# FeggieBoss/raytracing-course

Measured on AMD Instinct MI355X. Metric: Mray/s (closest-hit queries/s), dragon stand-in 1080p/256 spp, RAY_DEPTH 6, higher is better.
Workload: dtype f32

## Files before the change

raytracing-course_amd/csrc/device/pt_core.h:

```cpp
#pragma once
#include <stdint.h>

#if defined(__HIPCC__)
#include <hip/hip_runtime.h>
#define PT_HD __host__ __device__ __forceinline__
#else
#include <math.h>
#define PT_HD inline
#endif

namespace pt {

#if defined(__HIP_DEVICE_COMPILE__)
__device__ __forceinline__ bool pt_any(bool p) { return __ballot(p) != 0ull; }
#else
inline bool pt_any(bool p) { return p; }
#endif

struct f3 { float x, y, z; };
struct alignas(16) F4 { float x, y, z, w; };

PT_HD f3 mk3(float x, float y, float z) { f3 r; r.x = x; r.y = y; r.z = z; return r; }
PT_HD f3 operator+(f3 a, f3 b) { return mk3(a.x + b.x, a.y + b.y, a.z + b.z); }
PT_HD f3 operator-(f3 a, f3 b) { return mk3(a.x - b.x, a.y - b.y, a.z - b.z); }
PT_HD f3 operator*(f3 a, f3 b) { return mk3(a.x * b.x, a.y * b.y, a.z * b.z); }
PT_HD f3 operator/(f3 a, f3 b) { return mk3(a.x / b.x, a.y / b.y, a.z / b.z); }
PT_HD f3 operator*(float k, f3 a) { return mk3(k * a.x, k * a.y, k * a.z); }
PT_HD f3 operator*(f3 a, float k) { return mk3(a.x * k, a.y * k, a.z * k); }
PT_HD f3 operator/(f3 a, float k) { return mk3(a.x / k, a.y / k, a.z / k); }
PT_HD float dot(f3 a, f3 b) { return a.x * b.x + a.y * b.y + a.z * b.z; }
PT_HD f3 cross(f3 a, f3 b) { return mk3(a.y * b.z - b.y * a.z, a.z * b.x - b.z * a.x, a.x * b.y - b.x * a.y); }
PT_HD float fsqrt(float x) { return sqrtf(x); }
PT_HD f3 normalize(f3 v) { return v * (1.f / fsqrt(dot(v, v))); }
PT_HD float length(f3 v) { return fsqrt(dot(v, v)); }
PT_HD float smin(float a, float b) { return (b < a) ? b : a; }
PT_HD float smax(float a, float b) { return (a < b) ? b : a; }
PT_HD float fabs_(float a) { return fabsf(a); }

struct q4 { float x, y, z, w; };
PT_HD q4 conj(q4 q) { q4 r; r.x = -q.x; r.y = -q.y; r.z = -q.z; r.w = q.w; return r; }
PT_HD f3 qrot(q4 q, f3 v) {
    const f3 qv = mk3(q.x, q.y, q.z);
    const f3 uv = cross(qv, v);
    const f3 uuv = cross(qv, uv);
    return v + ((uv * q.w) + uuv) * 2.f;
}

#define PT_INF 1e18f
#define PT_PI_F 3.14159274101257324f

PT_HD uint32_t f2u(float f) { union { float f; uint32_t u; } c; c.f = f; return c.u; }
PT_HD float u2f(uint32_t u) { union { float f; uint32_t u; } c; c.u = u; return c.f; }

struct LogfEntry { double invc, logc; };
#if defined(__HIP_DEVICE_COMPILE__)
#define PT_TABLE __constant__
#else
#define PT_TABLE
#endif
PT_TABLE static const LogfEntry kLogfT[16] = {
    {0x1.661ec79f8f3bep+0, -0x1.57bf7808caadep-2}, {0x1.571ed4aaf883dp+0, -0x1.2bef0a7c06ddbp-2},
    {0x1.49539f0f010bp+0, -0x1.01eae7f513a67p-2},  {0x1.3c995b0b80385p+0, -0x1.b31d8a68224e9p-3},
    {0x1.30d190c8864a5p+0, -0x1.6574f0ac07758p-3}, {0x1.25e227b0b8eap+0, -0x1.1aa2bc79c81p-3},
    {0x1.1bb4a4a1a343fp+0, -0x1.a4e76ce8c0e5ep-4}, {0x1.12358f08ae5bap+0, -0x1.1973c5a611cccp-4},
    {0x1.0953f419900a7p+0, -0x1.252f438e10c1ep-5}, {0x1p+0, 0x0p+0},
    {0x1.e608cfd9a47acp-1, 0x1.aa5aa5df25984p-5},  {0x1.ca4b31f026aap-1, 0x1.c5e53aa362eb4p-4},
    {0x1.b2036576afce6p-1, 0x1.526e57720db08p-3},  {0x1.9c2d163a1aa2dp-1, 0x1.bc2860d22477p-3},
    {0x1.886e6037841edp-1, 0x1.1058bc8a07ee1p-2},  {0x1.767dcf5534862p-1, 0x1.4043057b6ee09p-2}};
PT_HD float logf_glibc(float x) {
    const double Ln2 = 0x1.62e42fefa39efp-1;
    const double A0 = -0x1.00ea348b88334p-2, A1 = 0x1.5575b0be00b6ap-2, A2 = -0x1.ffffef20a4123p-2;
    uint32_t ix = f2u(x);
    if (ix == 0x3f800000u) return 0.f;
    if (ix - 0x00800000u >= 0x7f800000u - 0x00800000u) {
        ix = f2u(x * 0x1p23f);
        ix -= 23u << 23;
    }
    const uint32_t tmp = ix - 0x3f330000u;
    const int i = (int)((tmp >> (23 - 4)) % 16u);
    const int k = (int32_t)tmp >> 23;
    const uint32_t iz = ix - (tmp & (0x1ffu << 23));
    const double invc = kLogfT[i].invc, logc = kLogfT[i].logc;
    const double z = (double)u2f(iz);
    const double r = z * invc - 1.0;
    const double y0 = logc + (double)k * Ln2;
    const double r2 = r * r;
    double y = A1 * r + A2;
    y = A0 * r2 + y;
    y = y * r2 + (y0 + r);
    return (float)y;
}

PT_HD double pow5_cr(double x) {
    const double x2 = x * x;
    const double h4 = x2 * x2;
    const double l4 = fma(x2, x2, -h4);
    const double h5 = h4 * x;
    const double e5 = fma(h4, x, -h5);
    return h5 + (e5 + l4 * x);
}

struct Rng {
    uint32_t x;
    float saved;
    uint32_t saved_ok;
};
PT_HD Rng rng_seed(uint32_t seed) {
    Rng r;
    const uint32_t s = seed % 2147483647u;
    r.x = (s == 0u) ? 1u : s;
    r.saved = 0.f;
    r.saved_ok = 0u;
    return r;
}
PT_HD uint32_t rng_next(Rng& r) {
    const uint64_t p = (uint64_t)r.x * 48271u;
    uint32_t v = (uint32_t)(p & 0x7fffffffu) + (uint32_t)(p >> 31);
    v = (v & 0x7fffffffu) + (v >> 31);
    if (v == 0x7fffffffu) v = 0u;
    r.x = v;
    return v;
}
PT_HD float rng_uniform(Rng& r) {
    const float sum = (float)(rng_next(r) - 1u);
    float u = sum / 2147483648.0f;
    if (u >= 1.0f) u = 0x1.fffffep-1f;
    return u * 1.0f + 0.0f;
}
PT_HD float rng_normal(Rng& r) {
    if (r.saved_ok) { r.saved_ok = 0u; return r.saved * 1.0f + 0.0f; }
    float a, b, r2;
    do {
        a = (float)((double)(2.0f * rng_uniform(r)) - 1.0);
        b = (float)((double)(2.0f * rng_uniform(r)) - 1.0);
        r2 = a * a + b * b;
    } while (r2 > 1.0f || r2 == 0.0f);
    const float m = fsqrt(-2.0f * logf_glibc(r2) / r2);
    r.saved = a * m;
    r.saved_ok = 1u;
    return b * m * 1.0f + 0.0f;
}

enum : uint32_t { T_PLANE = 1, T_BOX = 2, T_ELLIPSOID = 4, T_TRIANGLE = 8 };
enum : uint32_t { M_DIFFUSE = 0, M_METALLIC = 1, M_DIELECTRIC = 2 };

struct Node { F4 a, b; };
struct AuxNode { F4 a, b, c, d; };
#define PT_NODE_INTERIOR 0x80000000u
struct Prim { F4 p0, p1, p2, p3, p4; };
struct Shade { F4 s0, s1; };

struct SceneView {
    const Node* nodes;
    const AuxNode* aux;
    const Prim* prims;
    const Shade* shade;
    const uint32_t* planes;
    const uint32_t* emitters;
    uint32_t n_planes, n_emitters;
    f3 bg;
    float box_extent;
    const uint32_t* anc_info;
    const uint32_t* anc;
    const F4* blob;
    uint32_t o_nodes, o_aux, o_ainfo, o_anc, o_qprim, o_prim, o_bundle;
    uint32_t aux_rshift;
    float inv_emitters;
};

struct Ray { f3 o, d; };
struct Hit { float t; f3 n; uint32_t interior; };

PT_HD bool isect_plane(const Ray& r, f3 n, Hit& h) {
    const float dn = dot(r.d, n);
    const float t = -dot(r.o, n) / dn;
    if (t > 1e5f) return false;
    if (t > 0.f) {
        if (dn >= 0.f) { h.t = t; h.n = -1.f * n; h.interior = 1u; return true; }
        h.t = t; h.n = n; h.interior = 0u;
        return true;
    }
    return false;
}

PT_HD bool slab(f3 o, f3 d, f3 s, float& t, uint32_t& interior) {
    const f3 t1xyz = (-1.f * s - o) / d;
    const f3 t2xyz = (s - o) / d;
    const float t1x = smin(t1xyz.x, t2xyz.x), t2x = smax(t1xyz.x, t2xyz.x);
    const float t1y = smin(t1xyz.y, t2xyz.y), t2y = smax(t1xyz.y, t2xyz.y);
    const float t1z = smin(t1xyz.z, t2xyz.z), t2z = smax(t1xyz.z, t2xyz.z);
    const float t1 = smax(smax(t1x, t1y), t1z);
    const float t2 = smin(smin(t2x, t2y), t2z);
    if (t1 > t2) return false;
    if (t2 < 0.f) return false;
    interior = (t1 < 0.f) ? 1u : 0u;
    t = interior ? t2 : t1;
    return true;
}

PT_HD bool isect_box(const Ray& r, f3 s, Hit& h) {
    float t;
    uint32_t in;
    if (!slab(r.o, r.d, s, t, in)) return false;
    const f3 p = r.o + t * r.d;
    f3 n = p / s;
    if (in) n = -1.f * n;
    const float ax = fabs_(n.x), ay = fabs_(n.y), az = fabs_(n.z);
    float mx = ax;
    if (mx < ay) mx = ay;
    if (mx < az) mx = az;
    if (ax != mx) n.x = 0.f;
    if (ay != mx) n.y = 0.f;
    if (az != mx) n.z = 0.f;
    h.t = t; h.n = normalize(n); h.interior = in;
    return true;
}

PT_HD bool ellipsoid_root(const Ray& r, f3 rad, float& t, uint32_t& in) {
    const float a = dot(r.d / rad, r.d / rad);
    const float b = 2.f * dot(r.o / rad, r.d / rad);
    const float c = dot(r.o / rad, r.o / rad) - 1.f;
    const float d = b * b - 4.f * a * c;
    if (d <= 0.f) return false;
    const double sd = sqrt((double)d);
    float x1 = (float)(((double)-b - sd) / (double)(2.f * a));
    float x2 = (float)(((double)-b + sd) / (double)(2.f * a));
    if (x1 > x2) { const float tt = x1; x1 = x2; x2 = tt; }
    if (x2 < 0.f) return false;
    in = (x1 < 0.f) ? 1u : 0u;
    t = in ? x2 : x1;
    return true;
}
PT_HD bool isect_ellipsoid(const Ray& r, f3 rad, Hit& h) {
    float t;
    uint32_t in;
    if (!ellipsoid_root(r, rad, t, in)) return false;
    const f3 p = r.o + t * r.d;
    f3 n = normalize(p / (rad * rad));
    if (in) n = -1.f * n;
    h.t = t; h.n = n; h.interior = in;
    return true;
}

PT_HD bool isect_triangle_n(const Ray& r, f3 a, f3 b, f3 c, f3 n, Hit& h) {
    Hit ph;
    if (!isect_plane(r, n, ph)) return false;
    const f3 p = r.o + ph.t * r.d;
    if (!(dot(cross(b - a, p - a), n) > 0.f)) return false;
    if (!(dot(cross(p - a, c - a), n) > 0.f)) return false;
    if (!(dot(cross(c - b, p - b), n) > 0.f)) return false;
    h = ph;
    return true;
}
PT_HD bool isect_triangle(const Ray& r, f3 a, f3 b, f3 c, Hit& h) {
    return isect_triangle_n(r, a, b, c, normalize(cross(b - a, c - a)), h);
}

PT_HD bool prim_intersect(const Prim& P, const Ray& ray, Hit& h) {
    const f3 pos = mk3(P.p0.x, P.p0.y, P.p0.z);
    const uint32_t type = f2u(P.p0.w);
    q4 q; q.x = P.p1.x; q.y = P.p1.y; q.z = P.p1.z; q.w = P.p1.w;
    const q4 cq = conj(q);
    Ray lr;
    lr.o = qrot(cq, ray.o + -1.f * pos);
    lr.d = qrot(cq, ray.d);
    const f3 a = mk3(P.p2.x, P.p2.y, P.p2.z);
    bool ok;
    if (type == T_TRIANGLE) {
        ok = isect_triangle(lr, a, mk3(P.p3.x, P.p3.y, P.p3.z), mk3(P.p3.w, P.p4.x, P.p4.y), h);
    } else if (type == T_PLANE) {
        ok = isect_plane(lr, a, h);
    } else if (type == T_BOX) {
        ok = isect_box(lr, a, h);
    } else {
        ok = isect_ellipsoid(lr, a, h);
    }
    if (ok) h.n = normalize(qrot(q, h.n));
    return ok;
}

PT_HD bool bvh_prim_intersect(const Prim& P, const Ray& ray, Hit& h) {
    const f3 pos = mk3(P.p0.x, P.p0.y, P.p0.z);
    const uint32_t type = f2u(P.p0.w);
    q4 q; q.x = P.p1.x; q.y = P.p1.y; q.z = P.p1.z; q.w = P.p1.w;
    const q4 cq = conj(q);
    Ray lr;
    lr.o = qrot(cq, ray.o + -1.f * pos);
    lr.d = qrot(cq, ray.d);
    const f3 a = mk3(P.p2.x, P.p2.y, P.p2.z);
    bool ok;
    if (type == T_TRIANGLE) {
        ok = isect_triangle(lr, a, mk3(P.p3.x, P.p3.y, P.p3.z), mk3(P.p3.w, P.p4.x, P.p4.y), h);
    } else if (type == T_BOX) {
        ok = isect_box(lr, a, h);
    } else {
        ok = isect_ellipsoid(lr, a, h);
    }
    if (ok) h.n = normalize(qrot(q, h.n));
    return ok;
}

PT_HD bool plane_intersect(const Prim& P, const Ray& ray, Hit& h) {
    const f3 pos = mk3(P.p0.x, P.p0.y, P.p0.z);
    q4 q; q.x = P.p1.x; q.y = P.p1.y; q.z = P.p1.z; q.w = P.p1.w;
    const q4 cq = conj(q);
    Ray lr;
    lr.o = qrot(cq, ray.o + -1.f * pos);
    lr.d = qrot(cq, ray.d);
    if (!isect_plane(lr, mk3(P.p2.x, P.p2.y, P.p2.z), h)) return false;
    h.n = normalize(qrot(q, h.n));
    return true;
}

PT_HD f3 normal01_vec(Rng& R) {
    const float f1 = rng_normal(R);
    const float f2 = rng_normal(R);
    const float f3_ = rng_normal(R);
    return normalize(mk3(f1, f2, f3_));
}
PT_HD f3 sample_cosine(Rng& R, f3 n) {
    f3 dir = normal01_vec(R);
    dir = dir + n;
    if (dot(dir, n) <= 1e-8f) return n;
    if ((double)length(dir) <= 1e-4) return n;
    return normalize(dir);
}
PT_HD float pdf_cosine(f3 n, f3 d) { return smax(0.f, 1.f / PT_PI_F * dot(d, n)); }

PT_HD int points_for_pdf(const Prim& P, f3 x, f3 d, Hit& h1, Hit& h2) {
    Ray r; r.o = x; r.d = d;
    if (!prim_intersect(P, r, h1)) return 0;
    const float t = h1.t;
    if ((double)t <= 1e-8) return 0;
    const float eps = 1e-4f;
    Ray r2; r2.o = x + (t + eps) * d; r2.d = d;
    if (!prim_intersect(P, r2, h2)) return 1;
    h2.t += t + eps;
    return 2;
}

PT_HD f3 sample_box(Rng& R, const Prim& B, f3 x) {
    const f3 s = mk3(B.p2.x, B.p2.y, B.p2.z);
    const float wx = s.x * s.x, wy = s.y * s.y, wz = s.z * s.z;
    const f3 pos = mk3(B.p0.x, B.p0.y, B.p0.z);
    q4 q; q.x = B.p1.x; q.y = B.p1.y; q.z = B.p1.z; q.w = B.p1.w;
    for (;;) {
        float u = rng_uniform(R);
        const float side = (rng_uniform(R) <= 0.5f) ? 1.f : -1.f;
        u *= wx + wy + wz;
        float c1 = rng_uniform(R);
        float c2 = rng_uniform(R);
        float c3 = rng_uniform(R);
        c1 = 2.f * c1 - 1.f;
        c2 = 2.f * c2 - 1.f;
        c3 = 2.f * c3 - 1.f;
        f3 pnt = mk3(c1 * s.x, c2 * s.y, c3 * s.z);
        if (u < wx) pnt.x = side * s.x;
        else if (u < wx + wy) pnt.y = side * s.y;
        else pnt.z = side * s.z;
        const f3 on_box = qrot(q, pnt) + pos;
        const f3 smp = normalize(on_box - x);
        Hit h;
        Ray r; r.o = x; r.d = smp;
        if (prim_intersect(B, r, h)) return smp;
    }
}
PT_HD float pdf_point_box(const Prim& B, float dist2, f3 n, f3 d) {
    const float wx = B.p2.x * B.p2.x, wy = B.p2.y * B.p2.y, wz = B.p2.z * B.p2.z;
    const float p_y = 1.f / (8.f * (wx + wy + wz));
    return (p_y * dist2) / fabs_(dot(d, n));
}
PT_HD float pdf_box(const Prim& B, f3 x, f3 d) {
    Hit h1, h2;
    const int k = points_for_pdf(B, x, d, h1, h2);
    if (k == 0) return 1e-9f;
    const f3 cp = x + h1.t * d;
    float sum = pdf_point_box(B, dot(x - cp, x - cp), h1.n, d);
    if (k == 2) {
        const f3 op = x + h2.t * d;
        sum += pdf_point_box(B, dot(x - op, x - op), h2.n, d);
    }
    return sum;
}
PT_HD f3 sample_ellipsoid(Rng& R, const Prim& E, f3 x) {
    const f3 rr = mk3(E.p2.x, E.p2.y, E.p2.z);
    const f3 pos = mk3(E.p0.x, E.p0.y, E.p0.z);
    q4 q; q.x = E.p1.x; q.y = E.p1.y; q.z = E.p1.z; q.w = E.p1.w;
    for (;;) {
        const f3 k = normal01_vec(R);
        const f3 on = qrot(q, rr * k) + pos;
        const f3 smp = normalize(on - x);
        Hit h;
        Ray r; r.o = x; r.d = smp;
        if (prim_intersect(E, r, h)) return smp;
    }
}
PT_HD float pdf_point_ellipsoid(const Prim& E, float dist2, f3 y, f3 n_, f3 d) {
    const f3 rr = mk3(E.p2.x, E.p2.y, E.p2.z);
    const f3 pos = mk3(E.p0.x, E.p0.y, E.p0.z);
    q4 q; q.x = E.p1.x; q.y = E.p1.y; q.z = E.p1.z; q.w = E.p1.w;
    const f3 n = qrot(conj(q), y - pos) / rr;
    const float p_y = 1.f / (4.f * PT_PI_F * length(mk3(n.x * rr.y * rr.z, rr.x * n.y * rr.z, rr.x * rr.y * n.z)));
    return (p_y * dist2) / fabs_(dot(d, n_));
}
PT_HD float pdf_ellipsoid(const Prim& E, f3 x, f3 d) {
    Hit h1, h2;
    const int k = points_for_pdf(E, x, d, h1, h2);
    if (k == 0) return 1e-9f;
    const f3 cp = x + h1.t * d;
    float sum = pdf_point_ellipsoid(E, dot(x - cp, x - cp), cp, h1.n, d);
    if (k == 2) {
        const f3 op = x + h2.t * d;
        sum += pdf_point_ellipsoid(E, dot(x - op, x - op), op, h2.n, d);
    }
    return sum;
}
struct EmitGlobal {
    const SceneView& S;
    PT_HD Prim operator()(uint32_t k) const { return S.prims[S.emitters[k]]; }
};
template <class EM>
PT_HD f3 sample_mix_e(const SceneView& S, const EM& em, Rng& R, f3 x, f3 n) {
    const float flip = rng_uniform(R);
    if (S.n_emitters == 0u || flip <= 0.5f) return sample_cosine(R, n);
    const float fid = rng_uniform(R);
    const uint32_t id = (uint32_t)floorf(fid * (float)S.n_emitters);
    const Prim E = em(id);
    return f2u(E.p0.w) == T_BOX ? sample_box(R, E, x) : sample_ellipsoid(R, E, x);
}
PT_HD f3 sample_mix(const SceneView& S, Rng& R, f3 x, f3 n) { return sample_mix_e(S, EmitGlobal{S}, R, x, n); }
template <class EM>
PT_HD float pdf_mix_e(const SceneView& S, const EM& em, f3 x, f3 n, f3 d) {
    float sum = pdf_cosine(n, d);
    if (S.n_emitters != 0u) {
        float ps = 0.f;
        for (uint32_t k = 0; k < S.n_emitters; ++k) {
            const Prim E = em(k);
            ps += f2u(E.p0.w) == T_BOX ? pdf_box(E, x, d) : pdf_ellipsoid(E, x, d);
        }
        ps *= S.inv_emitters;
        sum = 0.5f * sum + 0.5f * ps;
    }
    return sum;
}
PT_HD float pdf_mix(const SceneView& S, f3 x, f3 n, f3 d) { return pdf_mix_e(S, EmitGlobal{S}, x, n, d); }

PT_HD f3 reflect(f3 n, f3 dir) { return dir - (2.0f * n) * dot(n, dir); }

PT_HD float saturate1(float v) { return smax(smin(1.f, v), 0.f); }
PT_HD float aces1(float x) {
    const float a = 2.51f, b = 0.03f, c = 2.43f, d = 0.59f, e = 0.14f;
    return saturate1((x * (a * x + b)) / (x * (c * x + d) + e));
}
PT_HD uint32_t quantize_gamma(float v, const float* thr) {
    uint32_t lo = 0;
    for (uint32_t step = 128; step >= 1; step >>= 1)
        if (thr[lo + step - 1] <= v) lo += step;
    return lo;
}

}
```

raytracing-course_amd/csrc/device/pt_trace.h:

```cpp
#pragma once
#include "pt_core.h"

namespace pt {

struct Counts {
    uint64_t rays;
    uint64_t nodes;
    uint64_t ptests;
    uint64_t planes;
    uint64_t aux;
    uint64_t fallbacks;
    uint32_t errs;
};

struct CamView {
    f3 pos, right, up, fwd;
    float tx, ty;
    float W, H;
};

PT_HD Ray camera_ray(const CamView& c, float x, float y) {
    const float nx = (2.f * x / c.W - 1.f) * c.tx;
    const float ny = -1.f * (2.f * y / c.H - 1.f) * c.ty;
    Ray r;
    r.o = c.pos;
    r.d = nx * c.right + ny * c.up + 1.f * c.fwd;
    return r;
}

#define PT_HITLIST 6

template <class Stack>
PT_HD int bvh_exact(const SceneView& S, const Ray& ray, float cb, Stack& stk, Hit& best, Counts& C) {
    int best_id = -1;
    best.t = PT_INF;
    float ms_t[PT_HITLIST];
    uint32_t ms_q[PT_HITLIST];
    uint32_t msn = 0;
    uint32_t nh = 0;
    uint32_t sp = 0;
    uint32_t node = 0;
    for (;;) {
        const Node nd = S.nodes[node];
        C.nodes++;
        const f3 c = mk3(nd.a.x, nd.a.y, nd.a.z);
        const f3 s = mk3(nd.a.w, nd.b.x, nd.b.y);
        float t;
        uint32_t interior;
        const bool hit = slab(ray.o + -1.f * c, ray.d, s, t, interior);
        bool descend = false;
        if (hit && !(cb < t && !interior)) {
            const uint32_t ref = f2u(nd.b.z), cnt = f2u(nd.b.w);
            if (!(cnt & PT_NODE_INTERIOR)) {
                Hit lb;
                lb.t = PT_INF;
                int lid = -1;
                for (uint32_t i = ref; i < ref + cnt; ++i) {
                    Hit h;
                    C.ptests++;
                    if (prim_intersect(S.prims[i], ray, h) && h.t < lb.t) { lb = h; lid = (int)i; }
                }
                if (lid >= 0) {
                    uint32_t keep = 0;
#pragma unroll
                    for (int k = 0; k < PT_HITLIST; ++k)
                        if ((uint32_t)k < msn && ms_t[k] < lb.t) keep = (uint32_t)k + 1u;
                    if (keep == PT_HITLIST) {
#pragma unroll
                        for (int k = 0; k + 1 < PT_HITLIST; ++k) { ms_t[k] = ms_t[k + 1]; ms_q[k] = ms_q[k + 1]; }
                        keep = PT_HITLIST - 1;
                        C.errs |= 1u;
                    }
#pragma unroll
                    for (int k = 0; k < PT_HITLIST; ++k)
                        if ((uint32_t)k == keep) { ms_t[k] = lb.t; ms_q[k] = nh; }
                    msn = keep + 1u;
                    nh++;
                    if (nh >= 255u) C.errs |= 2u;
                    if (lb.t < best.t) { best = lb; best_id = lid; }
                }
            } else {
                stk.set(sp++, ref | (nh << 24));
                node = node + 1u;
                descend = true;
            }
        }
        if (descend) continue;
        if (sp == 0u) break;
        const uint32_t e = stk.get(--sp);
        node = e & 0x00ffffffu;
        const uint32_t hs = e >> 24;
        if (hs != nh) {
            bool found = false;
#pragma unroll
            for (int k = 0; k < PT_HITLIST; ++k)
                if (!found && (uint32_t)k < msn && ms_q[k] >= hs) { cb = ms_t[k]; found = true; }
        }
    }
    return best_id;
}

#define PT_REPLAY_HITS 6

struct ReplayCfg {
    uint32_t as;
    uint32_t cap;
};

PT_HD bool aux_box(float lx, float ly, float lz, float hx, float hy, float hz, f3 inv, f3 oinv) {
    const float ax = fmaf(lx, inv.x, -oinv.x), bx = fmaf(hx, inv.x, -oinv.x);
    const float ay = fmaf(ly, inv.y, -oinv.y), by = fmaf(hy, inv.y, -oinv.y);
    const float az = fmaf(lz, inv.z, -oinv.z), bz = fmaf(hz, inv.z, -oinv.z);
    const float tn = fmaxf(fmaxf(fminf(ax, bx), fminf(ay, by)), fminf(az, bz));
    const float tf = fminf(fminf(fmaxf(ax, bx), fmaxf(ay, by)), fmaxf(az, bz));
    return tn <= tf && tf >= 0.f;
}

PT_HD bool node_slab(const Node& nd, const Ray& ray, float& t, uint32_t& interior) {
    const f3 c = mk3(nd.a.x, nd.a.y, nd.a.z);
    const f3 s = mk3(nd.a.w, nd.b.x, nd.b.y);
    return slab(ray.o + -1.f * c, ray.d, s, t, interior);
}

PT_HD void slab_approx(F4 a, F4 b, const Ray& ray, f3 rinv, float& t1, float& t2) {
    const f3 c = mk3(a.x, a.y, a.z);
    const f3 s = mk3(a.w, b.x, b.y);
    const f3 o = ray.o + -1.f * c;
    const f3 nlo = -1.f * s - o, nhi = s - o;
    const float ax = nlo.x * rinv.x, bx = nhi.x * rinv.x;
    const float ay = nlo.y * rinv.y, by = nhi.y * rinv.y;
    const float az = nlo.z * rinv.z, bz = nhi.z * rinv.z;
    t1 = smax(smax(smin(ax, bx), smin(ay, by)), smin(az, bz));
    t2 = smin(smin(smax(ax, bx), smax(ay, by)), smax(az, bz));
}

PT_HD uint32_t enter_decide(float t1, float t2, float bound) {
    const float e1 = fabsf(t1) * 0x1p-20f + 1e-30f, e2 = fabsf(t2) * 0x1p-20f + 1e-30f;
    const float d12 = t1 - t2;
    const float eb = 2.f * e1 + fabsf(bound) * 0x1p-22f;
    uint32_t v = bound < t1 ? 0u : 1u;
    v = fabsf(bound - t1) > eb ? v : 2u;
    v = t1 < 0.f ? 1u : v;
    v = fabsf(t1) > e1 ? v : 2u;
    v = t2 < 0.f ? 0u : v;
    v = fabsf(t2) > e2 ? v : 2u;
    v = d12 > 0.f ? 0u : v;
    v = (e1 < 1e20f && e2 < 1e20f) && fabsf(d12) > 2.f * (e1 + e2) ? v : 2u;
    return v;
}

PT_HD bool enter_exact(F4 a, F4 b, const Ray& ray, float bound) {
    const f3 c = mk3(a.x, a.y, a.z);
    const f3 s = mk3(a.w, b.x, b.y);
    float t;
    uint32_t in;
    if (!slab(ray.o + -1.f * c, ray.d, s, t, in)) return false;
    return !(bound < t && !in);
}

PT_HD bool node_enter(const Node& nd, const Ray& ray, f3 rinv, float bound, bool exact = false) {
    float t1, t2;
    slab_approx(nd.a, nd.b, ray, rinv, t1, t2);
    const uint32_t v = exact ? 2u : enter_decide(t1, t2, bound);
    if (v == 2u) return enter_exact(nd.a, nd.b, ray, bound);
    return v == 1u;
}

PT_HD bool aux_box_par(float lx, float ly, float lz, float hx, float hy, float hz, const Ray& r, f3 inv, f3 oinv) {
    const float lo[3] = {lx, ly, lz}, hi[3] = {hx, hy, hz};
    const float o[3] = {r.o.x, r.o.y, r.o.z}, d[3] = {r.d.x, r.d.y, r.d.z};
    const float iv[3] = {inv.x, inv.y, inv.z}, oi[3] = {oinv.x, oinv.y, oinv.z};
    float tn = -INFINITY, tf = INFINITY;
    bool inside = true;
#pragma unroll
    for (int k = 0; k < 3; ++k) {
        if (!(fabsf(d[k]) > 1e-30f)) {
            inside = inside && lo[k] <= o[k] && o[k] <= hi[k];
        } else {
            const float a = fmaf(lo[k], iv[k], -oi[k]), b = fmaf(hi[k], iv[k], -oi[k]);
            tn = fmaxf(tn, fminf(a, b));
            tf = fminf(tf, fmaxf(a, b));
        }
    }
    return inside && tn <= tf && tf >= 0.f;
}

PT_HD bool replay_ok_ray(const Ray& r) {
    const float m = 1e-30f, big = 3e38f;
    return fabsf(r.d.x) > m && fabsf(r.d.y) > m && fabsf(r.d.z) > m && fabsf(r.d.x) < big &&
           fabsf(r.d.y) < big && fabsf(r.d.z) < big && fabsf(r.o.x) < big && fabsf(r.o.y) < big &&
           fabsf(r.o.z) < big;
}

template <bool FAST, class Mem>
PT_HD int bvh_replay(const SceneView& S, const ReplayCfg& cfg, const Ray& ray, float P, Mem& L, Hit& best,
                     Counts& C, bool& fallback) {
    fallback = false;
    int best_id = -1;
    best.t = PT_INF;
    const f3 inv = mk3(1.f / ray.d.x, 1.f / ray.d.y, 1.f / ray.d.z);
    const f3 oinv = mk3(ray.o.x * inv.x, ray.o.y * inv.y, ray.o.z * inv.z);
    uint32_t h_idx[PT_REPLAY_HITS];
    float h_t[PT_REPLAY_HITS];
    uint32_t nh = 0;
    uint32_t lb = 0;
    for (;;) {
        uint32_t n = 0, mx = 0, mxpos = 0;
        bool overflow = false;
        uint32_t sp = 0;
        uint32_t node = 0;
        for (;;) {
            const AuxNode an = S.aux[node];
            C.aux++;
            const uint32_t c0 = f2u(an.d.x), c1 = f2u(an.d.y);
            const bool h0 = c0 != 0xffffffffu && aux_box(an.a.x, an.a.y, an.a.z, an.a.w, an.b.x, an.b.y, inv, oinv);
            const bool h1 = c1 != 0xffffffffu && aux_box(an.b.z, an.b.w, an.c.x, an.c.y, an.c.z, an.c.w, inv, oinv);
            uint32_t next = 0xffffffffu;
#pragma unroll
            for (int k = 0; k < 2; ++k) {
                const bool hk = k == 0 ? h0 : h1;
                const uint32_t code = k == 0 ? c0 : c1;
                if (!hk) continue;
                if (code & 0x80000000u) {
                    const uint32_t leaf = code & 0x7fffffffu;
                    if (leaf < lb) continue;
                    C.nodes++;
                    if (FAST) {
                        if (!node_enter(S.nodes[leaf], ray, inv, PT_INF)) continue;
                    } else {
                        float t;
                        uint32_t in;
                        if (!node_slab(S.nodes[leaf], ray, t, in)) continue;
                    }
                    if (n < cfg.cap) {
                        L.set(cfg.as + n, leaf);
                        if (leaf > mx || n == 0) { mx = leaf; mxpos = n; }
                        ++n;
                    } else {
                        overflow = true;
                        if (leaf < mx) {
                            L.set(cfg.as + mxpos, leaf);
                            mx = 0;
                            for (uint32_t q = 0; q < n; ++q) {
                                const uint32_t v = L.get(cfg.as + q);
                                if (v >= mx) { mx = v; mxpos = q; }
                            }
                        }
                    }
                } else if (next == 0xffffffffu) {
                    next = code;
                } else {
                    L.set(sp++, code);
                }
            }
            if (next != 0xffffffffu) { node = next; continue; }
            if (sp == 0u) break;
            node = L.get(--sp);
        }
        if (n == 0u) break;
        for (uint32_t i = 1; i < n; ++i) {
            const uint32_t v = L.get(cfg.as + i);
            uint32_t j = i;
            while (j > 0u) {
                const uint32_t u = L.get(cfg.as + j - 1u);
                if (u <= v) break;
                L.set(cfg.as + j, u);
                --j;
            }
            L.set(cfg.as + j, v);
        }
        uint32_t skip = lb;
        if (FAST) {
            uint32_t k = 0, cand = 0;
            while (k < n && (cand = L.get(cfg.as + k)) < skip) ++k;
            uint32_t a = 0;
            float bound = P;
            while (k < n) {
                const Node nd = S.nodes[a];
                C.nodes++;
                const uint32_t ref = f2u(nd.b.z), info = f2u(nd.b.w);
                bool next_cand = false;
                if (!node_enter(nd, ray, inv, bound)) {
                    skip = (info & PT_NODE_INTERIOR) ? (info & 0x7fffffffu) : a + 1u;
                    next_cand = true;
                } else if (a == cand) {
                    Hit lbh;
                    lbh.t = PT_INF;
                    int lid = -1;
                    for (uint32_t i = ref; i < ref + info; ++i) {
                        Hit h;
                        C.ptests++;
                        if (prim_intersect(S.prims[i], ray, h) && h.t < lbh.t) { lbh = h; lid = (int)i; }
                    }
                    if (lid >= 0) {
                        if (nh == PT_REPLAY_HITS) { fallback = true; return -1; }
#pragma unroll
                        for (int q = 0; q < PT_REPLAY_HITS; ++q)
                            if ((uint32_t)q == nh) { h_idx[q] = cand; h_t[q] = lbh.t; }
                        ++nh;
                        if (lbh.t < best.t) { best = lbh; best_id = lid; }
                    }
                    skip = cand + 1u;
                    next_cand = true;
                } else if (cand < ref) {
                    a = a + 1u;
                } else {
                    float m = bound;
                    bool any = false;
#pragma unroll
                    for (int q = 0; q < PT_REPLAY_HITS; ++q) {
                        if ((uint32_t)q < nh && h_idx[q] > a && h_idx[q] < ref) {
                            if (!any || h_t[q] < m) m = h_t[q];
                            any = true;
                        }
                    }
                    bound = m;
                    a = ref;
                }
                if (next_cand) {
                    ++k;
                    while (k < n && (cand = L.get(cfg.as + k)) < skip) ++k;
                    a = 0;
                    bound = P;
                }
            }
        } else {
            for (uint32_t k = 0; k < n; ++k) {
                const uint32_t cand = L.get(cfg.as + k);
                if (cand < skip) continue;
                uint32_t a = 0;
                float bound = P;
                for (;;) {
                    const Node nd = S.nodes[a];
                    C.nodes++;
                    float t;
                    uint32_t in;
                    const bool hit = node_slab(nd, ray, t, in);
                    const uint32_t ref = f2u(nd.b.z), info = f2u(nd.b.w);
                    if (!hit || (bound < t && !in)) {
                        skip = (info & PT_NODE_INTERIOR) ? (info & 0x7fffffffu) : a + 1u;
                        break;
                    }
                    if (a == cand) {
                        Hit lbh;
                        lbh.t = PT_INF;
                        int lid = -1;
                        for (uint32_t i = ref; i < ref + info; ++i) {
                            Hit h;
                            C.ptests++;
                            if (prim_intersect(S.prims[i], ray, h) && h.t < lbh.t) { lbh = h; lid = (int)i; }
                        }
                        if (lid >= 0) {
                            if (nh == PT_REPLAY_HITS) { fallback = true; return -1; }
#pragma unroll
                            for (int q = 0; q < PT_REPLAY_HITS; ++q)
                                if ((uint32_t)q == nh) { h_idx[q] = cand; h_t[q] = lbh.t; }
                            ++nh;
                            if (lbh.t < best.t) { best = lbh; best_id = lid; }
                        }
                        skip = cand + 1u;
                        break;
                    }
                    if (cand < ref) {
                        a = a + 1u;
                    } else {
                        float m = bound;
                        bool any = false;
#pragma unroll
                        for (int q = 0; q < PT_REPLAY_HITS; ++q) {
                            if ((uint32_t)q < nh && h_idx[q] > a && h_idx[q] < ref) {
                                if (!any || h_t[q] < m) m = h_t[q];
                                any = true;
                            }
                        }
                        bound = m;
                        a = ref;
                    }
                }
            }
        }
        if (!overflow) break;
        const uint32_t last = L.get(cfg.as + n - 1u) + 1u;
        lb = skip > last ? skip : last;
    }
    return best_id;
}

template <bool FAST, class Stack>
PT_HD int ray_intersection(const SceneView& S, const ReplayCfg& cfg, const Ray& ray, Stack& stk, Hit& out,
                           Counts& C) {
    int id = -1;
    float closest = PT_INF;
    for (uint32_t k = 0; k < S.n_planes; ++k) {
        const uint32_t pi = S.planes[k];
        Hit h;
        C.planes++;
        if (prim_intersect(S.prims[pi], ray, h) && h.t < closest) { closest = h.t; out = h; id = (int)pi; }
    }
    Hit bh;
    int bid;
    bool fallback = true;
    if (S.aux && replay_ok_ray(ray)) bid = bvh_replay<FAST>(S, cfg, ray, closest, stk, bh, C, fallback);
    if (fallback) {
        if (S.aux) C.fallbacks++;
        bid = bvh_exact(S, ray, closest, stk, bh, C);
    }
    if (bid != -1 && bh.t < closest) { out = bh; id = bid; }
    return id;
}

enum : uint32_t { V_TERM = 0u, V_DIFFUSE = 1u, V_COL = 2u, V_IDENT = 3u };

template <class EM>
PT_HD bool shade_vertex_e(const SceneView& S, const EM& em, const Shade& sh, Rng& R, Ray& ray, const Hit& h, int id,
                          uint32_t& idm, float& s1, float& s2) {
    const float eps = 1e-4f;
    const uint32_t mat = f2u(sh.s1.w);
    const f3 p = ray.o + h.t * ray.d;
    const f3 n = h.n;
    if (mat == M_DIFFUSE) {
        const f3 p_outer = p + eps * n;
        const f3 dir = sample_mix_e(S, em, R, p_outer, n);
        const float cosv = dot(dir, n);
        if (cosv <= 0.f) { idm = (uint32_t)id | (V_TERM << 30); s1 = s2 = 0.f; return false; }
        const float pw = pdf_mix_e(S, em, p_outer, n, dir);
        idm = (uint32_t)id | (V_DIFFUSE << 30);
        s1 = cosv;
        s2 = 1.f / pw;
        ray.o = p + eps * dir;
        ray.d = dir;
        return true;
    }
    if (mat == M_METALLIC) {
        const f3 rd = reflect(n, normalize(ray.d));
        idm = (uint32_t)id | (V_COL << 30);
        s1 = s2 = 1.f;
        ray.o = p + eps * rd;
        ray.d = rd;
        return true;
    }
    if (mat == M_DIELECTRIC) {
        float eta1 = 1.f, eta2 = sh.s0.w;
        if (h.interior) { const float tt = eta1; eta1 = eta2; eta2 = tt; }
        const f3 dir = -1.f * normalize(ray.d);
        const float cosn = dot(n, dir);
        const float sin2 = (float)((double)(eta1 / eta2) * sqrt((double)smax(0.f, 1.f - cosn * cosn)));
        bool refl;
        if (fabs((double)sin2) > 1.0) {
            refl = true;
        } else {
            const float q = (eta1 - eta2) / (eta1 + eta2);
            const float r0 = (float)((double)q * (double)q);
            const float rr = (float)((double)r0 + (double)(1.f - r0) * pow5_cr((double)(1.f - cosn)));
            refl = rng_uniform(R) < rr;
        }
        s1 = s2 = 1.f;
        if (refl) {
            const f3 rd = reflect(n, normalize(ray.d));
            idm = (uint32_t)id | (V_IDENT << 30);
            ray.o = p + eps * rd;
            ray.d = rd;
        } else {
            const float cos2 = (float)sqrt((double)(1.f - sin2 * sin2));
            const float k = eta1 / eta2;
            const f3 rd = k * (-1.f * dir) + (k * cosn - cos2) * n;
            idm = (uint32_t)id | ((h.interior ? V_IDENT : V_COL) << 30);
            ray.o = p + eps * rd;
            ray.d = rd;
        }
        return true;
    }
    idm = (uint32_t)id | (V_TERM << 30);
    s1 = s2 = 0.f;
    return false;
}
PT_HD bool shade_vertex(const SceneView& S, Rng& R, Ray& ray, const Hit& h, int id, uint32_t& idm, float& s1,
                        float& s2) {
    return shade_vertex_e(S, EmitGlobal{S}, S.shade[id], R, ray, h, id, idm, s1, s2);
}

PT_HD f3 fold_vertex_sh(const Shade& sh, f3 L, uint32_t idm, float s1, float s2) {
    const uint32_t mode = idm >> 30;
    const f3 E = mk3(sh.s1.x, sh.s1.y, sh.s1.z);
    f3 other;
    if (mode == V_TERM) {
        other = mk3(0.f, 0.f, 0.f);
    } else {
        const f3 col = mk3(sh.s0.x, sh.s0.y, sh.s0.z);
        f3 A;
        if (mode == V_DIFFUSE) A = col / PT_PI_F;
        else if (mode == V_COL) A = col;
        else A = mk3(1.f, 1.f, 1.f);
        other = ((A * L) * s1) * s2;
    }
    return E + other;
}
PT_HD f3 fold_vertex(const SceneView& S, f3 L, uint32_t idm, float s1, float s2) {
    return fold_vertex_sh(S.shade[idm & 0x3fffffffu], L, idm, s1, s2);
}

template <class Isect, class VStore>
PT_HD f3 trace_path_with(const SceneView& S, Isect&& isect, Ray ray, uint32_t depth, Rng& R, VStore& vs, Counts& C) {
    uint32_t nv = 0;
    f3 leaf = mk3(0.f, 0.f, 0.f);
    for (uint32_t rem = depth;; --rem) {
        if (rem == 0u) { leaf = mk3(0.f, 0.f, 0.f); break; }
        C.rays++;
        Hit h;
        const int id = isect(ray, h, C);
        if (id == -1) { leaf = S.bg; break; }
        uint32_t idm;
        float s1, s2;
        const bool cont = shade_vertex(S, R, ray, h, id, idm, s1, s2);
        vs.put(nv++, idm, s1, s2);
        if (!cont) break;
    }
    f3 L = leaf;
    while (nv > 0u) {
        --nv;
        uint32_t idm;
        float s1, s2;
        vs.get(nv, idm, s1, s2);
        L = fold_vertex(S, L, idm, s1, s2);
    }
    return L;
}

template <bool FAST, class Stack, class VStore>
PT_HD f3 trace_path(const SceneView& S, const ReplayCfg& cfg, Ray ray, uint32_t depth, Rng& R, Stack& stk, VStore& vs,
                    Counts& C) {
    return trace_path_with(
        S, [&](const Ray& r, Hit& h, Counts& c) { return ray_intersection<FAST>(S, cfg, r, stk, h, c); }, ray, depth, R,
        vs, C);
}

}
```

raytracing-course_amd/csrc/device/pt_wave.hip:

```cpp
#include "pt_wave.h"

namespace pt {

__global__ void __launch_bounds__(256) k_wcamera(WaveParams P) {
    const uint32_t t = P.tile_order ? P.tile_order[blockIdx.x] : blockIdx.x;
    const uint32_t slot = t * 256u + threadIdx.x;
    uint32_t x, y;
    const bool ok = slot_pixel(P.tm, t, threadIdx.x, x, y);
    bool want = false;
    Ray ray;
    if (ok) {
        PixelHot hot = load_hot(P.st, slot);
        Rng R = hot.R;
        uint32_t done = hot.done;
        if (P.depth == 0u) {
            f3 sum = load_sum(P.st, slot);
            for (; done < P.target; ++done) {
                (void)camera_sample(P.cam, R, x, y);
                sum = sum + mk3(0.f, 0.f, 0.f);
            }
            store_sum(P.st, slot, sum, y * P.tm.W + x);
        } else if (done < P.target) {
            ray = camera_sample(P.cam, R, x, y);
            want = true;
        }
        hot.R = R;
        hot.done = done;
        hot.nv = 0u;
        store_hot(P.st, slot, hot);
    }
    bool front = false;
    if (want) {
        const f3 rinv = mk3(1.f / ray.d.x, 1.f / ray.d.y, 1.f / ray.d.z);
        const f3 oinv = mk3(ray.o.x * rinv.x, ray.o.y * rinv.y, ray.o.z * rinv.z);
        for (uint32_t k = 0; k < PT_AUXW && k < P.n_top; ++k) {
            const AuxSL e = P.top[k];
            const uint32_t code = f2u(e.b.w);
            if (code == 0xffffffffu || !aux_box(e.a.x, e.a.y, e.a.z, e.a.w, e.b.x, e.b.y, rinv, oinv)) continue;
            if (code & 0x80000000u) {
                front = true;
                continue;
            }
            for (uint32_t j = 0; j < PT_AUXW; ++j) {
                const AuxSL c = P.top[code * PT_AUXW + j];
                front = front || (f2u(c.b.w) != 0xffffffffu && aux_box(c.a.x, c.a.y, c.a.z, c.a.w, c.b.x, c.b.y, rinv, oinv));
            }
        }
    }
    __shared__ uint32_t agg[5];
    uint32_t* ctl = P.ctl + PT_CTL_SET * P.parity;
    const uint32_t qf = block_append<4u>(ctl + C_FRONT, want && front, agg);
    const uint32_t qb = block_append<4u>(ctl + C_BACK, want && !front, agg);
    if (want) push_ray(P, front ? P.fq[P.parity] : P.fq[1u - P.parity], front ? qf : qb, ray, slot);
}

__global__ void __launch_bounds__(256) k_wcamera_merge(WaveParams P) {
    uint32_t* ctl = P.ctl + PT_CTL_SET * P.parity;
    const uint32_t nf = ctl[C_FRONT], nb = ctl[C_BACK];
    const RayQ A = P.fq[P.parity], B = P.fq[1u - P.parity];
    for (uint32_t i = blockIdx.x * 256u + threadIdx.x; i < nb; i += gridDim.x * 256u) {
        A.ro[nf + i] = B.ro[i];
        A.rd[nf + i] = B.rd[i];
        A.pid[nf + i] = B.pid[i];
        A.ri[nf + i] = B.ri[i];
    }
    if (blockIdx.x == 0u && threadIdx.x == 0u) ctl[C_FRESH] = nf + nb;
}

__device__ __forceinline__ uint32_t coop_order_bucket(const WaveParams& P, uint32_t gi, uint32_t n_carry) {
    const uint32_t done = P.st.rec[2u * work_item_slot(P, gi, n_carry)].w;
    const uint32_t rem = done < P.target ? P.target - done : 0u;
    const uint64_t b = (uint64_t)rem * PT_ORDER_BUCKETS / ((uint64_t)P.target + 1u);
    return PT_ORDER_BUCKETS - 1u - (uint32_t)b;
}
__global__ void __launch_bounds__(256) k_coop_hist(WaveParams P) {
    __shared__ uint32_t h[PT_ORDER_BUCKETS];
    const uint32_t* in = P.ctl + PT_CTL_SET * P.parity;
    const uint32_t n_carry = in[C_CARRY], n = in[C_FRESH] + n_carry;
    h[threadIdx.x] = 0u;
    __syncthreads();
    for (uint32_t gi = blockIdx.x * 256u + threadIdx.x; gi < n; gi += gridDim.x * 256u)
        atomicAdd(&h[coop_order_bucket(P, gi, n_carry)], 1u);
    __syncthreads();
    if (h[threadIdx.x]) atomicAdd(P.order_cur + PT_ORDER_BUCKETS + threadIdx.x, h[threadIdx.x]);
}
__global__ void __launch_bounds__(256) k_coop_scatter(WaveParams P) {
    __shared__ uint32_t base[PT_ORDER_BUCKETS];
    const uint32_t* in = P.ctl + PT_CTL_SET * P.parity;
    const uint32_t n_carry = in[C_CARRY], n = in[C_FRESH] + n_carry;
    if (threadIdx.x == 0u) {
        uint32_t t = 0u;
        for (uint32_t b = 0; b < PT_ORDER_BUCKETS; ++b) {
            base[b] = t;
            t += P.order_cur[PT_ORDER_BUCKETS + b];
        }
    }
    __syncthreads();
    for (uint32_t gi = blockIdx.x * 256u + threadIdx.x; gi < n; gi += gridDim.x * 256u) {
        const uint32_t b = coop_order_bucket(P, gi, n_carry);
        P.order[base[b] + atomicAdd(P.order_cur + b, 1u)] = gi;
    }
}

__global__ void __launch_bounds__(256) k_side_take(WaveParams P, uint32_t k, RayQ side, uint32_t* side_carry,
                                                   uint32_t* side_ctl) {
    const uint32_t* in = P.ctl + PT_CTL_SET * P.parity;
    const uint32_t n_carry = in[C_CARRY];
    const uint32_t j = blockIdx.x * 256u + threadIdx.x;
    const bool on = j < k;
    const uint32_t gi = on ? P.order[j] : 0u;
    const bool keep = on && P.drop != 1u + HO_SIDE_TAKE;
    wave_add_u64(ctr_copy(P.counters) + CTR_HO + HO_SIDE_TAKE, on ? 1ull : 0ull);
    const bool carry = keep && gi < n_carry;
    const uint32_t kc = wave_append(side_ctl + C_CARRY, carry);
    const uint32_t kf = wave_append(side_ctl + C_FRESH, keep && !carry);
    if (carry) {
        const auto rec = carry_rec(P.cq[P.parity], gi, P.carry_words);
        carry_put_restart(carry_rec(side_carry, kc, P.carry_words), rec.ray(), rec.slot());
    } else if (keep) {
        const RayQ& F = P.fq[P.parity];
        const uint32_t fi = gi - n_carry;
        side.ro[kf] = F.ro[fi];
        side.rd[kf] = F.rd[fi];
        side.pid[kf] = F.pid[fi];
        side.ri[kf] = F.ri[fi];
    }
}

__global__ void __launch_bounds__(64) k_wexact(WaveParams P) {
    extern __shared__ uint32_t lds_stack[];
    uint32_t* out = P.ctl + PT_CTL_SET * (1u - P.parity);
    const uint32_t n = out[C_EXACT];
    const uint32_t words = P.max_stack > P.aux_stack ? P.max_stack : P.aux_stack;
    LdsMemN<64u> stk{lds_stack + threadIdx.x, words, words};
    QCounts C{0u, 0u, 0u, 0u};
    uint32_t err = 0u;
    for (uint32_t k = blockIdx.x * 64u + threadIdx.x; k < n; k += gridDim.x * 64u) {
        const F4 o = P.ex.ro[k], d = P.ex.rd[k];
        Ray ray;
        ray.o = mk3(o.x, o.y, o.z);
        ray.d = mk3(d.x, d.y, d.z);
        Hit h;
        uint32_t used = 0u;
        const int id = q_run(P.S, ray, stk, h, C, used);
        err += C.planes >> 31;
        C.planes = 0u;
        const uint32_t j = f2u(d.w);
        P.done.ro[j] = o;
        P.done.rd[j] = F4{d.x, d.y, d.z, 0.f};
        P.done.id[j] = id < 0 ? 0xffffffffu : (uint32_t)id;
    }
    unsigned long long* ctr = ctr_copy(P.counters);
    wave_add_u64(ctr + 1, C.nodes);
    wave_add_u64(ctr + 2, C.ptests);
    wave_add_u64(ctr + 4, err);
}

__global__ void __launch_bounds__(256) k_wshade(WaveParams P) {
    __shared__ uint32_t agg[5];
    uint32_t* out = P.ctl + PT_CTL_SET * (1u - P.parity);
    const uint32_t n = out[C_EXACT];
    const RayQ N = P.fq[1u - P.parity];
    const uint32_t stride = gridDim.x * 256u;
    for (uint32_t base = blockIdx.x * 256u; base < n; base += stride) {
        const uint32_t i = base + threadIdx.x;
        bool emit = false, sdone = false;
        Ray ray;
        uint32_t slot = 0u;
        const uint32_t hid = i < n ? P.done.id[i] : PT_SUSPENDED;
        if (hid != PT_SUSPENDED) {
            const F4 o = P.done.ro[i], d = P.done.rd[i];
            slot = f2u(o.w);
            ray.o = mk3(o.x, o.y, o.z);
            ray.d = mk3(d.x, d.y, d.z);
            emit = shade_item(P, EmitGlobal{P.S}, slot, ray, hid, sdone);
        }
        if (P.progress) {
            const uint32_t nd = (uint32_t)__popcll(__ballot(sdone));
            if (nd && (threadIdx.x & 63u) == 0u)
                __hip_atomic_fetch_add(P.progress, (unsigned long long)nd, __ATOMIC_RELAXED, __HIP_MEMORY_SCOPE_SYSTEM);
        }
        const uint32_t qn = block_append<4u>(out + C_FRESH, emit, agg);
        if (emit) push_ray(P, N, qn, ray, slot);
    }
}

}

extern "C++" {
hipError_t pt_preload_kernels_wave() {
    hipFuncAttributes a;
    hipError_t e = hipFuncGetAttributes(&a, reinterpret_cast<const void*>(pt::k_wcamera));
    if (e == hipSuccess) e = pt_preload_kernels_path();
    if (e == hipSuccess) e = pt_preload_kernels_coop();
    return e;
}

hipError_t pt_launch_wave_start(pt::WaveParams p, hipStream_t s) {
    hipError_t e = hipMemsetAsync(p.ctl, 0, 4u * 2u * PT_CTL_SET, s);
    if (e != hipSuccess) return e;
    p.parity = 0u;
    hipLaunchKernelGGL(pt::k_wcamera, dim3(p.n_tiles_local), dim3(256), 0, s, p);
    hipLaunchKernelGGL(pt::k_wcamera_merge, dim3(p.n_tiles_local < 1024u ? p.n_tiles_local : 1024u), dim3(256), 0, s, p);
    return hipGetLastError();
}

hipError_t pt_launch_coop_order(pt::WaveParams p, uint32_t n, hipStream_t s) {
    hipError_t e = hipMemsetAsync(p.order_cur, 0, 2u * PT_ORDER_BUCKETS * 4u, s);
    if (e != hipSuccess) return e;
    const uint32_t grid = n / 256u + 1u < 1024u ? n / 256u + 1u : 1024u;
    hipLaunchKernelGGL(pt::k_coop_hist, dim3(grid), dim3(256), 0, s, p);
    hipLaunchKernelGGL(pt::k_coop_scatter, dim3(grid), dim3(256), 0, s, p);
    return hipGetLastError();
}

hipError_t pt_launch_side_take(pt::WaveParams p, uint32_t k, pt::RayQ side, uint32_t* side_carry, uint32_t* side_ctl,
                               hipStream_t s) {
    if (k == 0u) return hipSuccess;
    hipLaunchKernelGGL(pt::k_side_take, dim3((k + 255u) / 256u), dim3(256), 0, s, p, k, side, side_carry, side_ctl);
    return hipGetLastError();
}

hipError_t pt_launch_exact_shade(const pt::WaveParams& p, uint32_t shade_grid, hipStream_t s) {
    const uint32_t xw = p.max_stack > p.aux_stack ? p.max_stack : p.aux_stack;
    const uint32_t exact_lds = 64u * 4u * ((xw ? xw : 1u) + 1u);
    hipLaunchKernelGGL(pt::k_wexact, dim3(64), dim3(64), exact_lds, s, p);
    hipLaunchKernelGGL(pt::k_wshade, dim3(shade_grid), dim3(256), 0, s, p);
    return hipGetLastError();
}

}
```

Before: 4924.

## Reuse emitter-sampling hit in pdf, specialize solid intersect, inline polar normals

The accepted light-sample hit from sampling is kept and reused in the mixture pdf, so the first intersection with the chosen emitter is not recomputed. A box/ellipsoid-only intersect replaces the generic three-way primitive intersect. The Gaussian normal generator is inlined as explicit polar pairs with a saved spare, and sampling is restructured into one loop to reduce divergence. The shade kernel also gets a waves-per-EU occupancy hint, which may cause register spills.

```diff
diff --git a/raytracing-course_amd/csrc/device/pt_core.h b/raytracing-course_amd/csrc/device/pt_core.h
--- a/raytracing-course_amd/csrc/device/pt_core.h
+++ b/raytracing-course_amd/csrc/device/pt_core.h
@@ -300,6 +300,19 @@
     return ok;
 }
 
+PT_HD bool solid_intersect(const Prim& P, const Ray& ray, Hit& h) {
+    const f3 pos = mk3(P.p0.x, P.p0.y, P.p0.z);
+    q4 q; q.x = P.p1.x; q.y = P.p1.y; q.z = P.p1.z; q.w = P.p1.w;
+    const q4 cq = conj(q);
+    Ray lr;
+    lr.o = qrot(cq, ray.o + -1.f * pos);
+    lr.d = qrot(cq, ray.d);
+    const f3 a = mk3(P.p2.x, P.p2.y, P.p2.z);
+    const bool ok = f2u(P.p0.w) == T_BOX ? isect_box(lr, a, h) : isect_ellipsoid(lr, a, h);
+    if (ok) h.n = normalize(qrot(q, h.n));
+    return ok;
+}
+
 PT_HD bool plane_intersect(const Prim& P, const Ray& ray, Hit& h) {
     const f3 pos = mk3(P.p0.x, P.p0.y, P.p0.z);
     q4 q; q.x = P.p1.x; q.y = P.p1.y; q.z = P.p1.z; q.w = P.p1.w;
@@ -312,10 +325,38 @@
     return true;
 }
 
+PT_HD void polar_pair(Rng& r, float& am, float& bm) {
+    float a, b, r2;
+    do {
+        a = (float)((double)(2.0f * rng_uniform(r)) - 1.0);
+        b = (float)((double)(2.0f * rng_uniform(r)) - 1.0);
+        r2 = a * a + b * b;
+    } while (r2 > 1.0f || r2 == 0.0f);
+    const float m = fsqrt(-2.0f * logf_glibc(r2) / r2);
+    am = a * m;
+    bm = b * m;
+}
 PT_HD f3 normal01_vec(Rng& R) {
-    const float f1 = rng_normal(R);
-    const float f2 = rng_normal(R);
-    const float f3_ = rng_normal(R);
+    const bool had = R.saved_ok != 0u;
+    const float s0 = R.saved;
+    float am, bm;
+    polar_pair(R, am, bm);
+    float f1, f2, f3_;
+    if (had) {
+        f1 = s0 * 1.0f + 0.0f;
+        f2 = bm * 1.0f + 0.0f;
+        f3_ = am * 1.0f + 0.0f;
+        R.saved = am;
+        R.saved_ok = 0u;
+    } else {
+        float am2, bm2;
+        polar_pair(R, am2, bm2);
+        f1 = bm * 1.0f + 0.0f;
+        f2 = am * 1.0f + 0.0f;
+        f3_ = bm2 * 1.0f + 0.0f;
+        R.saved = am2;
+        R.saved_ok = 1u;
+    }
     return normalize(mk3(f1, f2, f3_));
 }
 PT_HD f3 sample_cosine(Rng& R, f3 n) {
@@ -327,52 +368,47 @@
 }
 PT_HD float pdf_cosine(f3 n, f3 d) { return smax(0.f, 1.f / PT_PI_F * dot(d, n)); }
 
-PT_HD int points_for_pdf(const Prim& P, f3 x, f3 d, Hit& h1, Hit& h2) {
-    Ray r; r.o = x; r.d = d;
-    if (!prim_intersect(P, r, h1)) return 0;
+struct EmitHit { Hit h; uint32_t id; bool ok; };
+PT_HD int points_for_pdf(const Prim& P, f3 x, f3 d, bool ok1, const Hit& h1, Hit& h2) {
+    if (!ok1) return 0;
     const float t = h1.t;
     if ((double)t <= 1e-8) return 0;
     const float eps = 1e-4f;
     Ray r2; r2.o = x + (t + eps) * d; r2.d = d;
-    if (!prim_intersect(P, r2, h2)) return 1;
+    if (!solid_intersect(P, r2, h2)) return 1;
     h2.t += t + eps;
     return 2;
 }
 
-PT_HD f3 sample_box(Rng& R, const Prim& B, f3 x) {
+PT_HD f3 box_candidate(Rng& R, const Prim& B, f3 x) {
     const f3 s = mk3(B.p2.x, B.p2.y, B.p2.z);
     const float wx = s.x * s.x, wy = s.y * s.y, wz = s.z * s.z;
     const f3 pos = mk3(B.p0.x, B.p0.y, B.p0.z);
     q4 q; q.x = B.p1.x; q.y = B.p1.y; q.z = B.p1.z; q.w = B.p1.w;
-    for (;;) {
-        float u = rng_uniform(R);
-        const float side = (rng_uniform(R) <= 0.5f) ? 1.f : -1.f;
-        u *= wx + wy + wz;
-        float c1 = rng_uniform(R);
-        float c2 = rng_uniform(R);
-        float c3 = rng_uniform(R);
-        c1 = 2.f * c1 - 1.f;
-        c2 = 2.f * c2 - 1.f;
-        c3 = 2.f * c3 - 1.f;
-        f3 pnt = mk3(c1 * s.x, c2 * s.y, c3 * s.z);
-        if (u < wx) pnt.x = side * s.x;
-        else if (u < wx + wy) pnt.y = side * s.y;
-        else pnt.z = side * s.z;
-        const f3 on_box = qrot(q, pnt) + pos;
-        const f3 smp = normalize(on_box - x);
-        Hit h;
-        Ray r; r.o = x; r.d = smp;
-        if (prim_intersect(B, r, h)) return smp;
-    }
+    float u = rng_uniform(R);
+    const float side = (rng_uniform(R) <= 0.5f) ? 1.f : -1.f;
+    u *= wx + wy + wz;
+    float c1 = rng_uniform(R);
+    float c2 = rng_uniform(R);
+    float c3 = rng_uniform(R);
+    c1 = 2.f * c1 - 1.f;
+    c2 = 2.f * c2 - 1.f;
+    c3 = 2.f * c3 - 1.f;
+    f3 pnt = mk3(c1 * s.x, c2 * s.y, c3 * s.z);
+    if (u < wx) pnt.x = side * s.x;
+    else if (u < wx + wy) pnt.y = side * s.y;
+    else pnt.z = side * s.z;
+    const f3 on_box = qrot(q, pnt) + pos;
+    return normalize(on_box - x);
 }
 PT_HD float pdf_point_box(const Prim& B, float dist2, f3 n, f3 d) {
     const float wx = B.p2.x * B.p2.x, wy = B.p2.y * B.p2.y, wz = B.p2.z * B.p2.z;
     const float p_y = 1.f / (8.f * (wx + wy + wz));
     return (p_y * dist2) / fabs_(dot(d, n));
 }
-PT_HD float pdf_box(const Prim& B, f3 x, f3 d) {
-    Hit h1, h2;
-    const int k = points_for_pdf(B, x, d, h1, h2);
+PT_HD float pdf_box(const Prim& B, f3 x, f3 d, bool ok1, const Hit& h1) {
+    Hit h2;
+    const int k = points_for_pdf(B, x, d, ok1, h1, h2);
     if (k == 0) return 1e-9f;
     const f3 cp = x + h1.t * d;
     float sum = pdf_point_box(B, dot(x - cp, x - cp), h1.n, d);
@@ -382,18 +418,13 @@
     }
     return sum;
 }
-PT_HD f3 sample_ellipsoid(Rng& R, const Prim& E, f3 x) {
+PT_HD f3 ellipsoid_candidate(Rng& R, const Prim& E, f3 x) {
     const f3 rr = mk3(E.p2.x, E.p2.y, E.p2.z);
     const f3 pos = mk3(E.p0.x, E.p0.y, E.p0.z);
     q4 q; q.x = E.p1.x; q.y = E.p1.y; q.z = E.p1.z; q.w = E.p1.w;
-    for (;;) {
-        const f3 k = normal01_vec(R);
-        const f3 on = qrot(q, rr * k) + pos;
-        const f3 smp = normalize(on - x);
-        Hit h;
-        Ray r; r.o = x; r.d = smp;
-        if (prim_intersect(E, r, h)) return smp;
-    }
+    const f3 k = normal01_vec(R);
+    const f3 on = qrot(q, rr * k) + pos;
+    return normalize(on - x);
 }
 PT_HD float pdf_point_ellipsoid(const Prim& E, float dist2, f3 y, f3 n_, f3 d) {
     const f3 rr = mk3(E.p2.x, E.p2.y, E.p2.z);
@@ -403,9 +434,9 @@
     const float p_y = 1.f / (4.f * PT_PI_F * length(mk3(n.x * rr.y * rr.z, rr.x * n.y * rr.z, rr.x * rr.y * n.z)));
     return (p_y * dist2) / fabs_(dot(d, n_));
 }
-PT_HD float pdf_ellipsoid(const Prim& E, f3 x, f3 d) {
-    Hit h1, h2;
-    const int k = points_for_pdf(E, x, d, h1, h2);
+PT_HD float pdf_ellipsoid(const Prim& E, f3 x, f3 d, bool ok1, const Hit& h1) {
+    Hit h2;
+    const int k = points_for_pdf(E, x, d, ok1, h1, h2);
     if (k == 0) return 1e-9f;
     const f3 cp = x + h1.t * d;
     float sum = pdf_point_ellipsoid(E, dot(x - cp, x - cp), cp, h1.n, d);
@@ -420,30 +451,58 @@
     PT_HD Prim operator()(uint32_t k) const { return S.prims[S.emitters[k]]; }
 };
 template <class EM>
-PT_HD f3 sample_mix_e(const SceneView& S, const EM& em, Rng& R, f3 x, f3 n) {
+PT_HD f3 sample_mix_e(const SceneView& S, const EM& em, Rng& R, f3 x, f3 n, EmitHit& eh) {
     const float flip = rng_uniform(R);
-    if (S.n_emitters == 0u || flip <= 0.5f) return sample_cosine(R, n);
-    const float fid = rng_uniform(R);
-    const uint32_t id = (uint32_t)floorf(fid * (float)S.n_emitters);
+    eh.h.t = 0.f; eh.h.n = mk3(0.f, 0.f, 0.f); eh.h.interior = 0u;
+    eh.id = 0xffffffffu;
+    eh.ok = false;
+    if (S.n_emitters == 0u) return sample_cosine(R, n);
+    const bool light = !(flip <= 0.5f);
+    f3 dir = n;
+    uint32_t id = 0u;
+    if (light) {
+        const float fid = rng_uniform(R);
+        id = (uint32_t)floorf(fid * (float)S.n_emitters);
+    } else {
+        dir = sample_cosine(R, n);
+    }
     const Prim E = em(id);
-    return f2u(E.p0.w) == T_BOX ? sample_box(R, E, x) : sample_ellipsoid(R, E, x);
-}
-PT_HD f3 sample_mix(const SceneView& S, Rng& R, f3 x, f3 n) { return sample_mix_e(S, EmitGlobal{S}, R, x, n); }
+    const bool box = f2u(E.p0.w) == T_BOX;
+    for (;;) {
+        if (light) dir = box ? box_candidate(R, E, x) : ellipsoid_candidate(R, E, x);
+        Ray r; r.o = x; r.d = dir;
+        eh.ok = solid_intersect(E, r, eh.h);
+        if (eh.ok || !light) break;
+    }
+    eh.id = id;
+    return dir;
+}
+PT_HD f3 sample_mix(const SceneView& S, Rng& R, f3 x, f3 n, EmitHit& eh) {
+    return sample_mix_e(S, EmitGlobal{S}, R, x, n, eh);
+}
 template <class EM>
-PT_HD float pdf_mix_e(const SceneView& S, const EM& em, f3 x, f3 n, f3 d) {
+PT_HD float pdf_mix_e(const SceneView& S, const EM& em, f3 x, f3 n, f3 d, const EmitHit& eh) {
     float sum = pdf_cosine(n, d);
     if (S.n_emitters != 0u) {
         float ps = 0.f;
         for (uint32_t k = 0; k < S.n_emitters; ++k) {
             const Prim E = em(k);
-            ps += f2u(E.p0.w) == T_BOX ? pdf_box(E, x, d) : pdf_ellipsoid(E, x, d);
+            Hit h1 = eh.h;
+            bool ok1 = eh.ok;
+            if (k != eh.id) {
+                Ray r; r.o = x; r.d = d;
+                ok1 = solid_intersect(E, r, h1);
+            }
+            ps += f2u(E.p0.w) == T_BOX ? pdf_box(E, x, d, ok1, h1) : pdf_ellipsoid(E, x, d, ok1, h1);
         }
         ps *= S.inv_emitters;
         sum = 0.5f * sum + 0.5f * ps;
     }
     return sum;
 }
-PT_HD float pdf_mix(const SceneView& S, f3 x, f3 n, f3 d) { return pdf_mix_e(S, EmitGlobal{S}, x, n, d); }
+PT_HD float pdf_mix(const SceneView& S, f3 x, f3 n, f3 d, const EmitHit& eh) {
+    return pdf_mix_e(S, EmitGlobal{S}, x, n, d, eh);
+}
 
 PT_HD f3 reflect(f3 n, f3 dir) { return dir - (2.0f * n) * dot(n, dir); }
 
diff --git a/raytracing-course_amd/csrc/device/pt_trace.h b/raytracing-course_amd/csrc/device/pt_trace.h
--- a/raytracing-course_amd/csrc/device/pt_trace.h
+++ b/raytracing-course_amd/csrc/device/pt_trace.h
@@ -420,10 +420,11 @@
     const f3 n = h.n;
     if (mat == M_DIFFUSE) {
         const f3 p_outer = p + eps * n;
-        const f3 dir = sample_mix_e(S, em, R, p_outer, n);
+        EmitHit eh;
+        const f3 dir = sample_mix_e(S, em, R, p_outer, n, eh);
         const float cosv = dot(dir, n);
         if (cosv <= 0.f) { idm = (uint32_t)id | (V_TERM << 30); s1 = s2 = 0.f; return false; }
-        const float pw = pdf_mix_e(S, em, p_outer, n, dir);
+        const float pw = pdf_mix_e(S, em, p_outer, n, dir, eh);
         idm = (uint32_t)id | (V_DIFFUSE << 30);
         s1 = cosv;
         s2 = 1.f / pw;
diff --git a/raytracing-course_amd/csrc/device/pt_wave.hip b/raytracing-course_amd/csrc/device/pt_wave.hip
--- a/raytracing-course_amd/csrc/device/pt_wave.hip
+++ b/raytracing-course_amd/csrc/device/pt_wave.hip
@@ -156,7 +156,7 @@
     wave_add_u64(ctr + 4, err);
 }
 
-__global__ void __launch_bounds__(256) k_wshade(WaveParams P) {
+__global__ void __launch_bounds__(256) __attribute__((amdgpu_waves_per_eu(5))) k_wshade(WaveParams P) {
     __shared__ uint32_t agg[5];
     uint32_t* out = P.ctl + PT_CTL_SET * (1u - P.parity);
     const uint32_t n = out[C_EXACT];
```

After: 4994 (median of 6 runs). +1.4%, better.
